# esw0116/DynaVSR

Hardware: AMD Instinct MI355X
Metric: inner-loop frames/sec/GPU (EDVR-M x4, 5x3x180x320): forward leg = BASELINE.json configs[1]; the inner MAML step and the per-frame pipeline are `inner_step` / `per_frame_pipeline` (higher is better)
Workload: dtype f32; 1 GPU; EDVR-M x4 forward (PCD deformable alignment + TSA fusion + reconstruction), clips of 1x5x3x180x320 -> 3x720x1280 (BASELINE.json configs[1]); one step = 2 clip(s) per GPU, one per HIP stream (adapt.super_resolve_video); clips_in_flight_per_gpu=2

## Files before the change

### dynavsr_amd/_lib.py

```python
import ctypes
import os
from ctypes import POINTER, Structure, c_char_p, c_float, c_int, c_longlong, c_size_t, c_void_p

import torch

_runtime = {"configured": False, "hw_queues": None, "effective": None}


def configure_runtime(hw_queues=6):
    if not _runtime["configured"]:
        user = os.environ.get("GPU_MAX_HW_QUEUES")
        late = torch.cuda.is_initialized()
        if user is None and not late:
            os.environ["GPU_MAX_HW_QUEUES"] = str(int(hw_queues))
        _runtime.update(configured=True, hw_queues=os.environ.get("GPU_MAX_HW_QUEUES"),
                        effective=(user is not None) or not late)
    return {"hw_queues": _runtime["hw_queues"], "effective": _runtime["effective"]}


def runtime_report(device=None):
    r = configure_runtime()
    overlaps = None
    if torch.cuda.is_available():
        with torch.cuda.device(device if device is not None else torch.cuda.current_device()):
# ... 126 lines not shown
        "dvsr_avgpool2_backward": (I, [P, P, LL, I, I, I, P]),
        "dvsr_resize_bilinear_ac_forward": (I, [P, P, LL, I, I, I, I, F, LL, P]),
        "dvsr_resize_bilinear_ac_backward": (I, [P, P, LL, I, I, I, I, F, LL, P]),
        "dvsr_upsample_bicubic_ac_forward": (I, [P, P, LL, I, I, I, P]),
        "dvsr_upsample_bicubic_ac_backward": (I, [P, P, LL, I, I, I, P]),
        "dvsr_channel_affine": (I, [P, P, P, P, I, I, LL, LL, LL, I, P]),
        "dvsr_batchnorm_workspace_bytes": (c_size_t, [I]),
        "dvsr_batchnorm_forward": (I, [P] * 8 + [I, I, LL, I, F, F, I, P, c_size_t, P]),
        "dvsr_batchnorm_backward": (I, [P] * 9 + [I, I, LL, I, I, P, c_size_t, P]),
        "dvsr_temporal_gather3_forward": (I, [P, P, I, I, I, LL, I, P]),
        "dvsr_temporal_gather3_backward": (I, [P, P, I, I, I, LL, I, P]),
        "dvsr_dynamic_filter_forward": (I, [P, P, P, P, I, I, I, I, I, P]),
        "dvsr_dynamic_filter_backward": (I, [P, P, P, P, P, P, I, I, I, I, I, P]),
        "dvsr_conv3x3_small_cout": (I, [P, P, P, P, P, I, I, I, I, I, I, P]),
        "dvsr_conv1x1_dual": (I, [P, P, P, P, P, P, P, I, I, I, I, I, P]),
        "dvsr_patch_gather_forward": (I, [P, P, POINTER(c_int), POINTER(c_int), I, I, I, I, I, I, P]),
        "dvsr_patch_gather_backward": (I, [P, P, POINTER(c_int), POINTER(c_int), I, I, I, I, I, I, P]),
        "dvsr_l1_tail_forward": (I, [P, P, P, F, P, LL, P, c_size_t, P]),
        "dvsr_l1_tail_backward": (I, [P, P, P, F, P, LL, P]),
        "dvsr_charbonnier_backward": (I, [P, P, P, P, LL, F, P]),
        "dvsr_charbonnier_forward_grouped": (I, [P, P, P, LL, I, F, P, c_size_t, P]),
        "dvsr_charbonnier_backward_grouped": (I, [P, P, P, P, LL, I, F, P]),
        "dvsr_l1_tail_forward_grouped": (I, [P, P, P, F, P, LL, I, P, c_size_t, P]),
        "dvsr_l1_tail_backward_grouped": (I, [P, P, P, F, P, LL, I, P]),
        "dvsr_edvr_op_info": (I, [P, I, c_char_p, I, c_char_p, I, POINTER(ctypes.c_double),
                                  POINTER(ctypes.c_double)]),
        "dvsr_edvr_forward_timed": (I, [P, POINTER(c_void_p), P, P, P, c_size_t, P, POINTER(c_float)]),
        "dvsr_debug_mfma_peak": (LL, [P, I, I, I, I, P]),
        "dvsr_debug_mfma_shadow": (I, [P, P, I, I, I, I, I, P]),
        "dvsr_edvr_tensor_info": (I, [P, c_char_p, POINTER(LL), POINTER(LL)]),
        "dvsr_edvr_plan_work": (I, [P, POINTER(ctypes.c_double * 9)]),
        "dvsr_edvr_plan_work_nograd": (I, [P, POINTER(ctypes.c_double * 9)]),
        "dvsr_edvr_op_launch_count": (I, [P, I, I]),
        "dvsr_side_stream_overlaps": (I, [P]),
        "dvsr_edvr_op_output": (I, [P, I, I, POINTER(c_int), POINTER(LL), POINTER(LL)]),
        "dvsr_estimator_plan_work": (I, [P, POINTER(ctypes.c_double * 9)]),
        "dvsr_edvr_stream_create": (I, [POINTER(EdvrConfig), I, I, I, POINTER(c_void_p)]),
        "dvsr_edvr_stream_destroy": (None, [P]),
        "dvsr_edvr_stream_num_params": (I, [P]),
        "dvsr_edvr_stream_num_launches": (I, [P, I]),
        "dvsr_edvr_stream_cache_bytes": (c_size_t, [P]),
        "dvsr_edvr_stream_workspace_bytes": (c_size_t, [P]),
        "dvsr_edvr_stream_extract": (I, [P, POINTER(c_void_p), P, I, P, c_size_t, P, c_size_t, I, P]),
        "dvsr_edvr_stream_fuse": (I, [P, POINTER(c_void_p), POINTER(c_int), P, c_size_t, P, P, c_size_t, I, P]),
        "dvsr_frame_ingest": (I, [P, POINTER(FrameDesc), P, I, I, I, P]),
        "dvsr_frame_emit": (I, [P, I, I, P, POINTER(FrameDesc), F, F, P]),
        "dvsr_edvr_stream_extract_frame": (I, [P, POINTER(c_void_p), P, POINTER(FrameDesc), I, I, P, c_size_t, P, c_size_t, I,
                                               P]),
# ... 54 lines not shown
```

### dynavsr_amd/csrc/engine.hip

```cpp
#include <algorithm>
#include <cstdlib>
#include <string>
#include <vector>

#include "common.h"
#include "kernels.h"
#include "small_grid.h"

namespace dvsr {

enum { SP_ARENA = 0, SP_INPUT = 1, SP_OUTPUT = 2, SP_NONE = 3 };
struct T {
  int space = SP_NONE;
  size_t off = 0, numel = 0;
  bool valid() const { return space != SP_NONE; }
};

enum OpType { OP_CONV, OP_DCN, OP_UP, OP_POOL, OP_GATE, OP_BLEND, OP_ADD, OP_PAD, OP_MEANSUB, OP_ADDMEAN };

struct Op {
  OpType type;
  const char* name = "";
  T x0, x1, res, y, y2;
  int pw = -1, pb = -1;
// ... 13 lines not shown
  float mul = 1.f;
  size_t planes = 0;
  int gB = 0, gN = 0, gC = 0;
  size_t gHW = 0;
  struct PackSlot { ConvGeo geo = {8, 8, 2}; size_t off = 0, floats = 0; };
  PackSlot dgrad[2], dcn_pack;
  enum LaunchRole { WHOLE, MAIN_PART, REF_PART };
  struct Launch { PackSlot pack; int c_off = 0, c = 0; LaunchRole role = WHOLE; };
  struct LaunchList {
    int n = 0; Launch l[2];
    const Launch* begin() const { return l; }
    const Launch* end() const { return l + n; }
    const Launch& primary() const { return l[n - 1]; }
  } launches[2];
  struct T pre;
};
enum FwdMode { FWD_GRAD = 0, FWD_NOGRAD = 1 };

enum { R_ACT = 0, R_GRAD = 1, R_X = 2, R_GX = 3, R_GOUT = 4, R_TMP = 5, R_NONE = 6 };
struct Ref {
  int space = R_NONE;
  size_t off = 0;
};
enum BType { B_MEMSET, B_COPYADD, B_ACT, B_WGRAD, B_DGRAD, B_REDUCE, B_DCN, B_UP, B_POOL, B_GATE, B_BLEND,
             B_PADFOLD, B_ADDMEAN, B_WUNMAP };
struct BOp {
  BType type;
  int fwd = -1;
  Ref a, b, c, d, e, f;
  size_t n = 0;
// ... 110 lines not shown
    if (g5.kernel == ConvKernel::WINO_F4) nograd.l[0] = whole(g5);
  }
  const Op::LaunchList pair = plan_hoist(o, p, fwd_ok, nograd.l[0]);
  if (pair.n) {
    o.pre = arena_alloc(p, "", (size_t)(N / o.x1_bdiv) * Cout * Ho * Wo);
    nograd = pair;
  }
  for (int which = 0; which < 2; ++which) {
    const int ci = which ? c1 : c0;
    if (!ci) continue;
    Op::PackSlot& dg = o.dgrad[which];
    dg.geo = as_bf(conv2_choose(ks, 1, N, o.H, o.W, ci, Cout, (!o.ps && o.stride == 1) ? ks_ok : ALLOW_NONE), o.H, o.W, ci, true);
    dg.floats = conv2_pack_floats(ks, ci, Cout, dg.geo);
    dg.off = p.dpack_floats;
    p.dpack_floats += dg.floats * p.wsets;
  }
}

struct Builder {
  dvsr_edvr_plan& p;
  int pcur = 0;
  explicit Builder(dvsr_edvr_plan& plan) : p(plan) {}

  T alloc(const char* name, size_t numel) { return arena_alloc(p, name, numel); }
  static T view(const T& base, size_t off, size_t numel) {
    T t = base;
    t.off += off;
    t.numel = numel;
    return t;
  }
// ... 147 lines not shown
  T emb = b.conv("tsa_emb", tA1, aligned, C, none, 0, BN, H, W, C, 3, 1, NO);
  T cor = b.alloc("tsa_cor", (size_t)BN * HW);
  T gated = b.alloc("tsa_gated", (size_t)BN * C * HW);
  {
    Op o; o.type = OP_GATE; o.name = "tsa_gate"; o.x0 = emb; o.x1 = emb_ref; o.res = aligned;
    o.y = cor; o.y2 = gated; o.gB = B; o.gN = Nf; o.gC = C; o.gHW = HW;
    p.ops.push_back(o);
  }
  T fea = b.conv("tsa_fea", ffu, gated, Nf * C, none, 0, B, H, W, C, 1, 1, L);
  T att = b.conv("tsa_att1", s1, gated, Nf * C, none, 0, B, H, W, C, 1, 1, L);
  {
    static const bool dual_on = [] { const char* v = getenv("DVSR_TSA_DUAL"); return !(v && v[0] == '0'); }();
    const int ia = (int)p.ops.size() - 2, ib = ia + 1;
    if (dual_on && C == 64 && !p.cfg.bf16_mfma) { p.ops[ia].dual = ib; p.ops[ib].fused_into = ia; }
  }
  T pmx, pav;
  b.pool("tsa_pool1", att, (size_t)B * C, H, W, pmx, pav);
  att = b.conv("tsa_att2", s2, pmx, C, pav, C, B, H2, W2, C, 1, 1, L);
  T attL = b.conv("tsa_attL1", sL1, att, C, none, 0, B, H2, W2, C, 1, 1, L);
  T qmx, qav;
  b.pool("tsa_pool2", attL, (size_t)B * C, H2, W2, qmx, qav);
  attL = b.conv("tsa_attL2", sL2, qmx, C, qav, C, B, H4, W4, C, 3, 1, L);
  attL = b.conv("tsa_attL3", sL3, attL, C, none, 0, B, H4, W4, C, 3, 1, L);
  T attLu = b.up("tsa_attL_up", attL, (size_t)B * C, H4, W4, 2, 1.f);
  T a3 = b.conv("tsa_att3", s3, att, C, none, 0, B, H2, W2, C, 3, 1, L);
  T att3 = b.alloc("tsa_att3_sum", (size_t)B * C * HW2);
  {
    Op o; o.type = OP_ADD; o.name = "tsa_att3_add"; o.x0 = a3; o.x1 = attLu; o.y = att3;
    p.ops.push_back(o);
  }
  T a4 = b.conv("tsa_att4", s4, att3, C, none, 0, B, H2, W2, C, 1, 1, L);
  T a4u = b.up("tsa_att4_up", a4, (size_t)B * C, H2, W2, 2, 1.f);
  T a5 = b.conv("tsa_att", s5, a4u, C, none, 0, B, H, W, C, 3, 1, NO);
  T ad = b.conv("tsa_add1", sa1, a5, C, none, 0, B, H, W, C, 1, 1, L);
  ad = b.conv("tsa_add2", sa2, ad, C, none, 0, B, H, W, C, 1, 1, NO);
  T out = b.alloc("tsa_out", (size_t)B * C * HW);
  {
    Op o; o.type = OP_BLEND; o.name = "tsa_blend"; o.x0 = fea; o.x1 = a5; o.res = ad; o.y = out;
    p.ops.push_back(o);
  }

  for (int i = 0; i < c.back_RBs; ++i) {
    auto p1 = b.take(); auto p2 = b.take();
    T t = b.conv("rc_rb_a", p1, out, C, none, 0, B, H, W, C, 3, 1, R);
    out = b.conv("rc_rb_b", p2, t, C, none, 0, B, H, W, C, 3, 1, NO, out);
  }
  p.named.emplace_back("recon", out);
  int h = H, w = W;
  if (c.scale == 4) {
    out = b.conv("upconv1", b.take(), out, C, none, 0, B, h, w, C * 4, 3, 1, L, none, 2);
    h *= 2; w *= 2;
    out = b.conv("upconv2", b.take(), out, C, none, 0, B, h, w, 256, 3, 1, L, none, 2);
  } else {
    out = b.conv("upconv2", b.take(), out, C, none, 0, B, h, w, 256, 3, 1, L, none, 2);
  }
// ... 431 lines not shown
        }
      }
    }
  }
  return flush();
}

static dvsr_conv2d_desc launch_desc(dvsr_conv2d_desc d, const Op& o, Op::LaunchRole role, float* pre) {
  if (role == Op::WHOLE) return d;
  if (role == Op::REF_PART) { d.x0 = d.x1; d.c0 = o.c1; d.x0_bstride = o.x1_bs; d.N = o.N / o.x1_bdiv; d.act = ACT_NONE; d.y = pre; }
  else { d.bias = nullptr; d.pre = pre; d.pre_bdiv = o.x1_bdiv; }
  d.x1 = nullptr; d.c1 = 0; d.x1_bdiv = 1; d.x1_bstride = 0;
  return d;
}

static int run_forward_op(const dvsr_edvr_plan& p, const Op& o, const float* const* P, const Bases& bs, hipStream_t st) {
  switch (o.type) {
    case OP_CONV: {
      dvsr_conv2d_desc d = {};
      d.x0 = bs.at(o.x0); d.x1 = bs.at(o.x1); d.w = P[o.pw]; d.bias = P[o.pb]; d.res = bs.at(o.res);
      d.y = bs.at(o.y);
      d.N = o.N; d.c0 = o.c0; d.c1 = o.c1; d.H = o.H; d.W = o.W; d.Cout = o.Cout; d.ks = o.ks;
      d.stride = o.stride; d.pad = conv_pad(o); d.act = o.act; d.pixel_shuffle = o.ps;
      if (o.pad_out) { d.y = bs.at(o.ypad); d.pixel_shuffle = o.pad_out; }
      if (!p.use_v1 && (o.dual >= 0 || o.fused_into >= 0)) {
        const Op& oa = o.dual >= 0 ? o : p.ops[o.fused_into];
        const Op& ob = p.ops[oa.dual];
        const long long HW = (long long)oa.H * oa.W;
        auto plain1x1 = [](const Op& q) {
          return q.type == OP_CONV && q.ks == 1 && q.stride == 1 && q.c1 == 0 && q.Cout == 64 && !q.res.valid() && !q.ps && !q.wmap && !q.pad_out;
        };
// ... 310 lines not shown
  {
    const ConvGeo& g = p->ops[index].launches[FWD_NOGRAD].primary().pack.geo;
    snprintf(name, name_cap, "%s[%d/%d/%d%s]", p->ops[index].name, g.cc, g.th, g.mt, kernel_tag(g.kernel));
  }
  else
    snprintf(name, name_cap, "%s", p->ops[index].name);
  return DVSR_OK;
}

extern "C" int dvsr_edvr_op_launch_count(const dvsr_edvr_plan* p, int index, int nograd) {
  if (!p || index < 0 || index >= (int)p->ops.size()) return -1;
  const Op& o = p->ops[index];
  return o.type == OP_CONV ? o.launches[nograd ? FWD_NOGRAD : FWD_GRAD].n : 1;
}

static int plan_work(const dvsr_edvr_plan* p, double* out9, FwdMode mode) {
  DVSR_REQUIRE(p && out9, DVSR_ERR_INVALID, "edvr_plan_work: null argument");
  double fa = 0, fe = 0, ba = 0, be = 0, fby = 0, f32p[2] = {0, 0}, bfp[2] = {0, 0};
  auto conv_part = [](const Op& o, int ci) {
    return 2.0 * (double)o.N * conv_out(o, o.H) * conv_out(o, o.W) * o.Cout * ci * o.ks * o.ks;
  };
  auto issue = [&](const ConvGeo& g, double f, double* ex, int pass) {
    const double shaped = f * multiplies_per_output_ratio(g.kernel);
    *ex += shaped;
    if (on_bf16_split(g.kernel) || g.bf == 2) bfp[pass] += 6.0 * shaped;
    else if (g.bf == 1) bfp[pass] += shaped;
    else f32p[pass] += shaped;
  };
  for (const Op& o : p->ops) {
    {
      const char* k; double fl, by;
      op_work(o, &k, &fl, &by);
      fby += by;
    }
    if (o.type == OP_CONV) {
      const double f = conv_part(o, o.c0 + o.c1);
      fa += f;
      for (const Op::Launch& l : o.launches[mode])
        issue(l.pack.geo, conv_part(o, l.c) / (l.role == Op::REF_PART ? o.x1_bdiv : 1), &fe, 0);
    } else if (o.type == OP_DCN) {
      const double f = 2.0 * (double)o.N * o.H * o.W * o.Cout * o.c0 * 9;
      fa += f; fe += f; f32p[0] += f;
    }
  }
  for (const BOp& b : p->bops) {
    if (b.fwd < 0) continue;
    const Op& o = p->ops[b.fwd];
// ... 407 lines not shown
```

### dynavsr_amd/csrc/kernels.h

```cpp
#pragma once
#include "../../include/dynavsr_hip.h"
#include "common.h"

namespace dvsr {

struct ConvExtra {
  int wt = 0;
  int w_ctot = 0, w_coff = 0;
  int in_ps = 0;
  int in_dil = 0, Hs = 0, Ws = 0;
  int accum = 0;
  const float* gmask = nullptr;
  int gmask_act = 0;
  int wdiv = 1; long long w_gs = 0; int b_gs = 0;
};
int conv2d_run(const dvsr_conv2d_desc& d, const ConvExtra& ex, hipStream_t st);

int mdcn_forward_run(const float* x, const float* off, long long off_bs, const float* msk,
                     long long msk_bs, int mask_logit, const float* w, const float* b, float* out,
                     int N, int C, int H, int W, int Cout, int kh, int kw, int stride, int pad,
                     int dil, int groups, int dg, int act, hipStream_t st);

enum class ConvKernel : int {
  REG = 0,
// ... 57 lines not shown
  return conv2_pack_entry(w, P, ks, Cout, Ctot, g.cc, g.bf, pack_layout(g.kernel), wt, w_ctot, w_coff);
}
double conv2_f4_occupied_cycles(int N, int Ho, int Wo, int Cout, int Ctot, int th);
int pack_weights_wino_run(const PackTable& t, hipStream_t st);
int pack_weights_wino3_run(const PackTable& t, hipStream_t st);
int pack_weights_wino5_run(const PackTable& t, hipStream_t st);
int conv2d_packed_run(const dvsr_conv2d_desc& d, const float* wp, const ConvExtra& ex, const ConvGeo& geo,
                      hipStream_t st);

bool conv1x1_dual_ok(const float* x, const float* w0, const float* w1, const float* y0, const float* y1, int Cin, long long HW);
int conv1x1_dual_run(const float* x, const float* w0, const float* b0, const float* w1, const float* b1, float* y0, float* y1,
                     int N, int Cin, int HW, int act, hipStream_t st, int wdiv = 1, long long w_gs = 0, int b_gs = 0);
int conv3x3_small_cout_run(const float* x, const float* w, const float* bias, const float* res, float* y, int N,
                           int C, int H, int W, int Cout, int act, hipStream_t st, int wdiv = 1, long long w_gs = 0,
                           int b_gs = 0);

struct WgradReduceEntry {
  float* partial; float* dbp; float* dW; float* db;
  int nslot, KK, OP, CP, Cout, Cin, Ctot, c_off;
  int ngroups = 1;
  long long dW_gs = 0, db_gs = 0;
};
constexpr int WGRAD_REDUCE_BATCH = 44;
struct WgradReduceTable {
  int n;
  WgradReduceEntry e[WGRAD_REDUCE_BATCH];
};
int wgrad_reduce_batch(const WgradReduceEntry* entries, int n, hipStream_t st, int blocks = 96);
struct WgradDesc {
  const float* x = nullptr; long long x_bs = 0; int x_bdiv = 1;
// ... 143 lines not shown
```

### dynavsr_amd/engine.py

```python
import ctypes
import threading

import torch

from . import _lib as L

_plans = {}
_GEOMETRY_ENV = ("DVSR_CONV_WINO", "DVSR_CONV_WINO3", "DVSR_CONV_WINO5", "DVSR_CONV_V1", "DVSR_EST_SPLIT", "DVSR_EST_SPLIT2", "DVSR_FUSE_ACT_BWD",
                 "DVSR_BWD_STREAMS", "DVSR_PCD_HOIST")
_PROCESS_ENV = ("DVSR_CONV_LDS", "DVSR_CONV_LAST_MFMA", "DVSR_SPLIT_TH8_FROM", "DVSR_WGRAD_SPLIT3",
                "DVSR_WGRAD_WIDE", "DVSR_WGRAD_S3V", "DVSR_WGRAD_S3_KYS_BELOW", "DVSR_WGRAD_S3_WGS", "DVSR_WGRAD_S3W", "DVSR_DCN_FWD", "DVSR_DCN_BWD",
                "DVSR_EST_FUSE_PAD", "DVSR_FUSE_RES_BWD", "DVSR_BWD_FORK_EVERY", "DVSR_BWD_PROBE", "DVSR_TSA_DUAL", "DVSR_TSA_V",
                "DVSR_DEGRADE_GENERIC", "DVSR_UP2")
_process_env_seen = None


def _check_process_env():
    import os
    import warnings
    global _process_env_seen
    now = tuple(os.environ.get(k) for k in _PROCESS_ENV)
    if _process_env_seen is None:
        _process_env_seen = now
        return
# ... 63 lines not shown
        L.check(L.lib().dvsr_edvr_op_output(self._h, index, which, ctypes.byref(ia), ctypes.byref(off), ctypes.byref(n)),
                "dvsr_edvr_op_output")
        if not ia.value:
            return None
        return ws.view(torch.float32)[off.value:off.value + n.value]

    def op_info(self):
        out = []
        kind, name = ctypes.create_string_buffer(32), ctypes.create_string_buffer(64)
        fl, by = ctypes.c_double(), ctypes.c_double()
        for i in range(self.n_launches):
            L.check(L.lib().dvsr_edvr_op_info(self._h, i, kind, 32, name, 64, ctypes.byref(fl),
                                              ctypes.byref(by)), "dvsr_edvr_op_info")
            out.append((kind.value.decode(), name.value.decode(), fl.value, by.value))
        return out

    def tensor(self, ws, name, shape=None):
        off, n = ctypes.c_longlong(), ctypes.c_longlong()
        L.check(L.lib().dvsr_edvr_tensor_info(self._h, name.encode(), ctypes.byref(off),
                                              ctypes.byref(n)), "dvsr_edvr_tensor_info")
        t = ws.view(torch.float32)[off.value:off.value + n.value]
        return t.view(shape) if shape is not None else t

    def __del__(self):
        try:
            if self._h:
                L.lib().dvsr_edvr_plan_destroy(self._h)
        except Exception:
            pass

# ... 415 lines not shown
```

### include/dynavsr_hip.h

```cpp
#ifndef DYNAVSR_HIP_H_
#define DYNAVSR_HIP_H_

#include <stddef.h>

#ifdef __cplusplus
extern "C" {
#endif

#define DVSR_OK 0
#define DVSR_ERR_INVALID (-1)
#define DVSR_ERR_UNSUPPORTED (-2)
#define DVSR_ERR_WORKSPACE (-3)
#define DVSR_ERR_HIP (-4)

#define DVSR_ACT_NONE 0
#define DVSR_ACT_LRELU 1
#define DVSR_ACT_RELU 2

typedef void* dvsr_stream_t;

const char* dvsr_last_error(void);
int dvsr_version(void);

int dvsr_mdcn_forward(const float* x, const float* offset, const float* mask, const float* w,
// ... 78 lines not shown
int dvsr_edvr_num_launches(const dvsr_edvr_plan* plan);
size_t dvsr_edvr_workspace_bytes(const dvsr_edvr_plan* plan, int need_grad);
int dvsr_edvr_forward(const dvsr_edvr_plan* plan, const float* const* params, const float* x,
                      float* out, void* workspace, size_t workspace_bytes, dvsr_stream_t stream);
int dvsr_edvr_forward_packed(const dvsr_edvr_plan* plan, const float* const* params, const float* x,
                             float* out, void* workspace, size_t workspace_bytes, dvsr_stream_t stream);
int dvsr_edvr_backward(const dvsr_edvr_plan* plan, const float* const* params, const float* x,
                       const float* grad_out, float* const* grad_params, float* grad_x, void* workspace,
                       size_t workspace_bytes, dvsr_stream_t stream);
int dvsr_edvr_num_backward_launches(const dvsr_edvr_plan* plan);
int dvsr_edvr_op_info(const dvsr_edvr_plan* plan, int index, char* kind, int kind_cap, char* name,
                      int name_cap, double* flops, double* bytes);
int dvsr_edvr_plan_work(const dvsr_edvr_plan* plan, double* out9);
int dvsr_edvr_plan_work_nograd(const dvsr_edvr_plan* plan, double* out9);
int dvsr_edvr_op_launch_count(const dvsr_edvr_plan* plan, int index, int nograd);
int dvsr_side_stream_overlaps(dvsr_stream_t stream);
int dvsr_edvr_op_output(const dvsr_edvr_plan* plan, int index, int which, int* in_arena, long long* offset_floats,
                        long long* numel);
int dvsr_edvr_forward_timed(const dvsr_edvr_plan* plan, const float* const* params, const float* x,
                            float* out, void* workspace, size_t workspace_bytes,
                            dvsr_stream_t stream, float* op_ms);
long long dvsr_debug_mfma_peak(float* out, int blocks, int iters, int nacc, int lds_bytes, dvsr_stream_t stream);
int dvsr_debug_mfma_shadow(long long* cycles, float* out, int blocks, int iters, int nv, int kind, int acc,
                           dvsr_stream_t stream);
int dvsr_edvr_tensor_info(const dvsr_edvr_plan* plan, const char* name, long long* offset_floats,
                          long long* numel);

#define DVSR_STREAM_MAX_FRAMES 16
typedef struct dvsr_edvr_stream dvsr_edvr_stream;
int dvsr_edvr_stream_create(const dvsr_edvr_config* cfg, int H, int W, int slots, dvsr_edvr_stream** out);
// ... 175 lines not shown
                                  dvsr_stream_t stream);
int dvsr_temporal_gather3_backward(const float* grad_y, float* grad_x, int B, int T, int C, long long HW, int pad_t,
                                   dvsr_stream_t stream);
int dvsr_dynamic_filter_forward(const float* x_center, const float* filter_logits, const float* residual, float* out,
                                int B, int H, int W, int scale, int adapt_official, dvsr_stream_t stream);
int dvsr_dynamic_filter_backward(const float* x_center, const float* filter_logits, const float* grad_out,
                                 float* grad_logits, float* grad_residual, float* grad_x_center, int B, int H, int W,
                                 int scale, int adapt_official, dvsr_stream_t stream);

int dvsr_conv3x3_small_cout(const float* x, const float* w, const float* bias, const float* res, float* y, int N, int C, int H,
                            int W, int Cout, int act, dvsr_stream_t stream);

int dvsr_conv1x1_dual(const float* x, const float* w0, const float* b0, const float* w1, const float* b1, float* y0, float* y1,
                      int N, int Cin, int H, int W, int act, dvsr_stream_t stream);

int dvsr_patch_gather_forward(const float* src, float* dst, const int* py, const int* px, int P, int planes, int H, int W,
                              int edge, int scale, dvsr_stream_t stream);
int dvsr_patch_gather_backward(const float* grad_dst, float* grad_src, const int* py, const int* px, int P, int planes,
                               int H, int W, int edge, int scale, dvsr_stream_t stream);

int dvsr_adam_step(float* const* params, const float* const* grads, float* const* exp_avg,
                   float* const* exp_avg_sq, const long long* numel, int n_tensors, float lr, float beta1,
                   float beta2, float eps, float weight_decay, int step, dvsr_stream_t stream);
int dvsr_sgd_step(float* const* params, const float* const* grads, const long long* numel, int n_tensors,
                  float lr, float weight_decay, dvsr_stream_t stream);
int dvsr_replicate_tensors(const float* const* src, float* const* dst, const long long* numel, int n_tensors, int copies,
                           dvsr_stream_t stream);

size_t dvsr_frame_metrics_workspace_bytes(int C, int H, int W);
int dvsr_frame_metrics(const float* sr, const float* gt, int C, int H, int W, float lo, float hi,
// ... 11 lines not shown
```

Before: 266.0 frames/s.

## Fuse TSA pool/attention, upsample-add/attention and tail convs into MFMA kernels

Adds three fused HIP kernels for the TSA fusion module. The first does pool plus two 1x1 convs, the second does bilinear upsample-add plus a 1x1 conv, and the third does the add1/add2 1x1 convs plus the sigmoid blend. The planner marks the absorbed ops and, in no-grad forward mode, launches one fused kernel per chain instead of several separate ones. The aim is to cut launches and the round trips of intermediate activations through global memory. It only applies for nf=64, fp32 and aligned shapes, can be turned off with DVSR_TSA_FUSE=0, and leaves the grad forward path unchanged.

```diff
diff --git a/dynavsr_amd/_lib.py b/dynavsr_amd/_lib.py
--- a/dynavsr_amd/_lib.py
+++ b/dynavsr_amd/_lib.py
@@ -164,6 +164,9 @@
         "dvsr_dynamic_filter_backward": (I, [P, P, P, P, P, P, I, I, I, I, I, P]),
         "dvsr_conv3x3_small_cout": (I, [P, P, P, P, P, I, I, I, I, I, I, P]),
         "dvsr_conv1x1_dual": (I, [P, P, P, P, P, P, P, I, I, I, I, I, P]),
+        "dvsr_tsa_pool_att": (I, [P, P, P, P, P, P, P, I, I, I, P]),
+        "dvsr_tsa_up_add_att": (I, [P, P, P, P, P, I, I, I, P]),
+        "dvsr_tsa_tail": (I, [P, P, P, P, P, P, P, I, I, I, P]),
         "dvsr_patch_gather_forward": (I, [P, P, POINTER(c_int), POINTER(c_int), I, I, I, I, I, I, P]),
         "dvsr_patch_gather_backward": (I, [P, P, POINTER(c_int), POINTER(c_int), I, I, I, I, I, I, P]),
         "dvsr_l1_tail_forward": (I, [P, P, P, F, P, LL, P, c_size_t, P]),
@@ -182,6 +185,7 @@
         "dvsr_edvr_plan_work": (I, [P, POINTER(ctypes.c_double * 9)]),
         "dvsr_edvr_plan_work_nograd": (I, [P, POINTER(ctypes.c_double * 9)]),
         "dvsr_edvr_op_launch_count": (I, [P, I, I]),
+        "dvsr_edvr_op_absorbed_by": (I, [P, I]),
         "dvsr_side_stream_overlaps": (I, [P]),
         "dvsr_edvr_op_output": (I, [P, I, I, POINTER(c_int), POINTER(LL), POINTER(LL)]),
         "dvsr_estimator_plan_work": (I, [P, POINTER(ctypes.c_double * 9)]),
diff --git a/dynavsr_amd/csrc/engine.hip b/dynavsr_amd/csrc/engine.hip
--- a/dynavsr_amd/csrc/engine.hip
+++ b/dynavsr_amd/csrc/engine.hip
@@ -51,6 +51,8 @@
     const Launch& primary() const { return l[n - 1]; }
   } launches[2];
   struct T pre;
+  enum TsaChain { CHAIN_NONE = 0, CHAIN_POOL_ATT, CHAIN_UP_ADD_ATT, CHAIN_TAIL };
+  int tsa_chain = CHAIN_NONE, absorbed_by = -1, chain_ops[2] = {-1, -1};
 };
 enum FwdMode { FWD_GRAD = 0, FWD_NOGRAD = 1 };
 
@@ -191,6 +193,29 @@
     dg.floats = conv2_pack_floats(ks, ci, Cout, dg.geo);
     dg.off = p.dpack_floats;
     p.dpack_floats += dg.floats * p.wsets;
+  }
+}
+
+static bool tsa_chain_applies(const dvsr_edvr_plan& p, Op::TsaChain which) {
+  const char* v = getenv("DVSR_TSA_FUSE");
+  if ((v && v[0] == '0') || p.use_v1 || p.wsets != 1 || p.cfg.nf != 64 || p.cfg.bf16_mfma || p.H % 4 != 0 || p.W % 4 != 0) return false;
+  return which != Op::CHAIN_UP_ADD_ATT || (p.W / 4) % 4 == 0;
+}
+static void plan_tsa_chain(dvsr_edvr_plan& p, Op::TsaChain which, int a, int b, int last) {
+  if (!tsa_chain_applies(p, which)) return;
+  p.ops[last].tsa_chain = which;
+  p.ops[last].chain_ops[0] = a; p.ops[last].chain_ops[1] = b;
+  p.ops[a].absorbed_by = p.ops[b].absorbed_by = p.ops[last].absorbed_by = last;
+}
+static double tsa_chain_bytes(const dvsr_edvr_plan& p, const Op& last) {
+  const Op& a = p.ops[last.chain_ops[0]];
+  const Op& b = p.ops[last.chain_ops[1]];
+  auto wts = [](const Op& c) { return (double)c.Cout * (c.c0 + c.c1); };
+  switch (last.tsa_chain) {
+    case Op::CHAIN_POOL_ATT: return 4.0 * ((double)a.planes * a.H * a.W + (double)b.y.numel + (double)last.y.numel + wts(b) + wts(last));
+    case Op::CHAIN_UP_ADD_ATT: return 4.0 * ((double)a.planes * a.H * a.W + (double)b.x0.numel + (double)last.y.numel + wts(last));
+    case Op::CHAIN_TAIL: return 4.0 * (3.0 * last.y.numel + wts(a) + wts(b));
+    default: return 0.0;
   }
 }
 
@@ -368,15 +393,19 @@
     const int ia = (int)p.ops.size() - 2, ib = ia + 1;
     if (dual_on && C == 64 && !p.cfg.bf16_mfma) { p.ops[ia].dual = ib; p.ops[ib].fused_into = ia; }
   }
+  auto last_op = [&]() { return (int)p.ops.size() - 1; };
   T pmx, pav;
   b.pool("tsa_pool1", att, (size_t)B * C, H, W, pmx, pav);
+  const int i_pool1 = last_op();
   att = b.conv("tsa_att2", s2, pmx, C, pav, C, B, H2, W2, C, 1, 1, L);
   T attL = b.conv("tsa_attL1", sL1, att, C, none, 0, B, H2, W2, C, 1, 1, L);
+  plan_tsa_chain(p, Op::CHAIN_POOL_ATT, i_pool1, last_op() - 1, last_op());
   T qmx, qav;
   b.pool("tsa_pool2", attL, (size_t)B * C, H2, W2, qmx, qav);
   attL = b.conv("tsa_attL2", sL2, qmx, C, qav, C, B, H4, W4, C, 3, 1, L);
   attL = b.conv("tsa_attL3", sL3, attL, C, none, 0, B, H4, W4, C, 3, 1, L);
   T attLu = b.up("tsa_attL_up", attL, (size_t)B * C, H4, W4, 2, 1.f);
+  const int i_attL_up = last_op();
   T a3 = b.conv("tsa_att3", s3, att, C, none, 0, B, H2, W2, C, 3, 1, L);
   T att3 = b.alloc("tsa_att3_sum", (size_t)B * C * HW2);
   {
@@ -384,6 +413,7 @@
     p.ops.push_back(o);
   }
   T a4 = b.conv("tsa_att4", s4, att3, C, none, 0, B, H2, W2, C, 1, 1, L);
+  plan_tsa_chain(p, Op::CHAIN_UP_ADD_ATT, i_attL_up, last_op() - 1, last_op());
   T a4u = b.up("tsa_att4_up", a4, (size_t)B * C, H2, W2, 2, 1.f);
   T a5 = b.conv("tsa_att", s5, a4u, C, none, 0, B, H, W, C, 3, 1, NO);
   T ad = b.conv("tsa_add1", sa1, a5, C, none, 0, B, H, W, C, 1, 1, L);
@@ -393,6 +423,7 @@
     Op o; o.type = OP_BLEND; o.name = "tsa_blend"; o.x0 = fea; o.x1 = a5; o.res = ad; o.y = out;
     p.ops.push_back(o);
   }
+  plan_tsa_chain(p, Op::CHAIN_TAIL, last_op() - 2, last_op() - 1, last_op());
 
   for (int i = 0; i < c.back_RBs; ++i) {
     auto p1 = b.take(); auto p2 = b.take();
@@ -854,7 +885,36 @@
   return d;
 }
 
+static int tsa_chain_launch(const dvsr_edvr_plan& p, const Op& last, const float* const* P, const Bases& bs, hipStream_t st, bool run,
+                            bool* ok) {
+  const Op& a = p.ops[last.chain_ops[0]];
+  const Op& b = p.ops[last.chain_ops[1]];
+  switch (last.tsa_chain) {
+    case Op::CHAIN_POOL_ATT:
+      *ok = tsa_pool_att_ok(P[b.pw], P[last.pw], b.Cout, a.H, a.W);
+      return run ? tsa_pool_att_run(bs.at(a.x0), P[b.pw], P[b.pb], P[last.pw], P[last.pb], bs.at(b.y), bs.at(last.y), b.N, a.H, a.W, st)
+                 : DVSR_OK;
+    case Op::CHAIN_UP_ADD_ATT:
+      *ok = tsa_up_add_att_ok(bs.at(a.x0), P[last.pw], last.Cout, last.H, last.W);
+      return run ? tsa_up_add_att_run(bs.at(b.x0), bs.at(a.x0), P[last.pw], P[last.pb], bs.at(last.y), last.N, last.H, last.W, st)
+                 : DVSR_OK;
+    case Op::CHAIN_TAIL:
+      *ok = tsa_tail_ok(bs.at(a.x0), bs.at(last.x0), P[a.pw], P[b.pw], bs.at(last.y), a.Cout, (long long)a.H * a.W);
+      return run ? tsa_tail_run(bs.at(a.x0), bs.at(last.x0), P[a.pw], P[a.pb], P[b.pw], P[b.pb], bs.at(last.y), a.N, a.H * a.W, st)
+                 : DVSR_OK;
+    default:
+      *ok = false;
+      return DVSR_OK;
+  }
+}
+
 static int run_forward_op(const dvsr_edvr_plan& p, const Op& o, const float* const* P, const Bases& bs, hipStream_t st) {
+  if (bs.mode == FWD_NOGRAD && o.absorbed_by >= 0) {
+    const Op& last = p.ops[o.absorbed_by];
+    bool ok = false;
+    (void)tsa_chain_launch(p, last, P, bs, st, false, &ok);
+    if (ok) return &o == &last ? tsa_chain_launch(p, last, P, bs, st, true, &ok) : DVSR_OK;
+  }
   switch (o.type) {
     case OP_CONV: {
       dvsr_conv2d_desc d = {};
@@ -1195,6 +1255,11 @@
   return o.type == OP_CONV ? o.launches[nograd ? FWD_NOGRAD : FWD_GRAD].n : 1;
 }
 
+extern "C" int dvsr_edvr_op_absorbed_by(const dvsr_edvr_plan* p, int index) {
+  if (!p || index < 0 || index >= (int)p->ops.size()) return -2;
+  return p->ops[index].absorbed_by;
+}
+
 static int plan_work(const dvsr_edvr_plan* p, double* out9, FwdMode mode) {
   DVSR_REQUIRE(p && out9, DVSR_ERR_INVALID, "edvr_plan_work: null argument");
   double fa = 0, fe = 0, ba = 0, be = 0, fby = 0, f32p[2] = {0, 0}, bfp[2] = {0, 0};
@@ -1212,6 +1277,7 @@
     {
       const char* k; double fl, by;
       op_work(o, &k, &fl, &by);
+      if (mode == FWD_NOGRAD && o.absorbed_by >= 0) by = &o == &p->ops[o.absorbed_by] ? tsa_chain_bytes(*p, o) : 0.0;
       fby += by;
     }
     if (o.type == OP_CONV) {
diff --git a/dynavsr_amd/csrc/kernels.h b/dynavsr_amd/csrc/kernels.h
--- a/dynavsr_amd/csrc/kernels.h
+++ b/dynavsr_amd/csrc/kernels.h
@@ -95,6 +95,16 @@
 int conv3x3_small_cout_run(const float* x, const float* w, const float* bias, const float* res, float* y, int N,
                            int C, int H, int W, int Cout, int act, hipStream_t st, int wdiv = 1, long long w_gs = 0,
                            int b_gs = 0);
+
+bool tsa_pool_att_ok(const float* w2, const float* wl, int C, int H, int W);
+int tsa_pool_att_run(const float* x, const float* w2, const float* b2, const float* wl, const float* bl, float* att, float* attl,
+                     int N, int H, int W, hipStream_t st);
+bool tsa_up_add_att_ok(const float* al, const float* w, int C, int H, int W);
+int tsa_up_add_att_run(const float* a3, const float* al, const float* w, const float* b, float* y, int N, int H, int W,
+                       hipStream_t st);
+bool tsa_tail_ok(const float* a5, const float* fea, const float* w1, const float* w2, const float* out, int C, long long HW);
+int tsa_tail_run(const float* a5, const float* fea, const float* w1, const float* b1, const float* w2, const float* b2,
+                 float* out, int N, int HW, hipStream_t st);
 
 struct WgradReduceEntry {
   float* partial; float* dbp; float* dW; float* db;
diff --git a/dynavsr_amd/csrc/tsa_fused.hip b/dynavsr_amd/csrc/tsa_fused.hip
--- /dev/null
+++ b/dynavsr_amd/csrc/tsa_fused.hip
@@ -0,0 +1,306 @@
+#include "common.h"
+#include "kernels.h"
+
+namespace dvsr {
+namespace {
+
+constexpr int TF_C = 64;
+
+template <int K>
+__device__ __forceinline__ void load_w_row(const float* __restrict__ w, int co, int hi, float (&a)[K / 2]) {
+#pragma unroll
+  for (int m = 0; m < K / 4; ++m) {
+    const f32x4 v = *reinterpret_cast<const f32x4*>(w + (size_t)co * K + 4 * m);
+    a[2 * m] = hi ? v[1] : v[0];
+    a[2 * m + 1] = hi ? v[3] : v[2];
+  }
+}
+
+__device__ __forceinline__ int acc_row(int r, int hi) { return (r & 3) + 8 * (r >> 2) + 4 * hi; }
+
+__device__ __forceinline__ void load_bias(const float* __restrict__ b, int cw, int hi, float (&bv)[16]) {
+#pragma unroll
+  for (int r = 0; r < 16; ++r) bv[r] = b ? b[cw + acc_row(r, hi)] : 0.f;
+}
+
+template <int K, int NJ, int PITCH>
+__device__ __forceinline__ void contract(const float* s, const float (&a)[K / 2], f32x16 (&acc)[NJ]) {
+#pragma unroll
+  for (int j = 0; j < NJ; ++j)
+#pragma unroll
+    for (int r = 0; r < 16; ++r) acc[j][r] = 0.f;
+#pragma unroll
+  for (int i = 0; i < K / 2; ++i) {
+    if constexpr (NJ == 2) {
+      const f32x2 b = *reinterpret_cast<const f32x2*>(s + 2 * i * PITCH);
+      acc[0] = __builtin_amdgcn_mfma_f32_32x32x2f32(a[i], b[0], acc[0], 0, 0, 0);
+      acc[1] = __builtin_amdgcn_mfma_f32_32x32x2f32(a[i], b[1], acc[1], 0, 0, 0);
+    } else {
+      acc[0] = __builtin_amdgcn_mfma_f32_32x32x2f32(a[i], s[2 * i * PITCH], acc[0], 0, 0, 0);
+    }
+  }
+}
+
+__device__ __forceinline__ float lrelu(float v) { return fmaxf(v, 0.1f * v); }
+
+constexpr int TP_PX = 64;
+
+struct TsaPoolAttK {
+  const float* x; const float* w2; const float* b2; const float* wl; const float* bl; float* att; float* attl;
+  int H, W, Ho, Wo, tiles_per_img;
+};
+
+__global__ __launch_bounds__(256) void tsa_pool_att_kernel(TsaPoolAttK a) {
+  __shared__ __attribute__((aligned(16))) float s_x[2 * TF_C * TP_PX];
+  __shared__ __attribute__((aligned(16))) float s_t[TF_C * TP_PX];
+  const int tile = blockIdx.x;
+  const int n = tile / a.tiles_per_img, p0 = (tile - n * a.tiles_per_img) * TP_PX;
+  const int tid = threadIdx.x, lane = tid & 63;
+  const int wave = __builtin_amdgcn_readfirstlane(tid >> 6);
+  const int nn = lane & 31, hi = lane >> 5, cw = (wave & 1) * 32, ph = wave >> 1;
+  const int HWo = a.Ho * a.Wo;
+
+  float a2[TF_C], al[TF_C / 2], bv2[16], bvl[16];
+  load_w_row<2 * TF_C>(a.w2, cw + nn, hi, a2);
+  load_w_row<TF_C>(a.wl, cw + nn, hi, al);
+  load_bias(a.b2, cw, hi, bv2);
+  load_bias(a.bl, cw, hi, bvl);
+
+  {
+    const int pl = tid & 63;
+    const int p = min(p0 + pl, HWo - 1);
+    const int oy = p / a.Wo, ox = p - oy * a.Wo;
+    int toff[9];
+    bool tin[9];
+#pragma unroll
+    for (int t = 0; t < 9; ++t) {
+      const int yy = 2 * oy + t / 3 - 1, xx = 2 * ox + t % 3 - 1;
+      tin[t] = (unsigned)yy < (unsigned)a.H && (unsigned)xx < (unsigned)a.W;
+      toff[t] = min(max(yy, 0), a.H - 1) * a.W + min(max(xx, 0), a.W - 1);
+    }
+    const float* xn = a.x + (size_t)n * TF_C * a.H * a.W;
+#pragma unroll 4
+    for (int k = 0; k < TF_C / 4; ++k) {
+      const int c = (tid >> 6) + 4 * k;
+      const float* pln = xn + (size_t)c * a.H * a.W;
+      float v[9];
+#pragma unroll
+      for (int t = 0; t < 9; ++t) v[t] = pln[toff[t]];
+      float mx = -INFINITY, sum = 0.f;
+#pragma unroll
+      for (int t = 0; t < 9; ++t) {
+        mx = fmaxf(mx, tin[t] ? v[t] : -INFINITY);
+        sum += tin[t] ? v[t] : 0.f;
+      }
+      s_x[c * TP_PX + pl] = mx;
+      s_x[(TF_C + c) * TP_PX + pl] = sum * (1.f / 9.f);
+    }
+  }
+  __syncthreads();
+
+  const int col = ph * 32 + nn, px = p0 + col;
+  const bool live = px < HWo;
+  f32x16 acc[1];
+  contract<2 * TF_C, 1, TP_PX>(s_x + hi * TP_PX + col, a2, acc);
+  float* yb = a.att + (size_t)n * TF_C * HWo + px;
+#pragma unroll
+  for (int r = 0; r < 16; ++r) {
+    const int co = cw + acc_row(r, hi);
+    const float v = lrelu(acc[0][r] + bv2[r]);
+    s_t[co * TP_PX + col] = v;
+    if (live) yb[(size_t)co * HWo] = v;
+  }
+  __syncthreads();
+  contract<TF_C, 1, TP_PX>(s_t + hi * TP_PX + col, al, acc);
+  yb = a.attl + (size_t)n * TF_C * HWo + px;
+  if (live) {
+#pragma unroll
+    for (int r = 0; r < 16; ++r) yb[(size_t)(cw + acc_row(r, hi)) * HWo] = lrelu(acc[0][r] + bvl[r]);
+  }
+}
+
+struct TsaUpAddAttK {
+  const float* a3; const float* al; const float* w; const float* b; float* y;
+  int H, W, tiles_per_img;
+};
+
+__global__ __launch_bounds__(256) void tsa_up_add_att_kernel(TsaUpAddAttK a) {
+  __shared__ __attribute__((aligned(16))) float s_x[TF_C * TP_PX];
+  const int tile = blockIdx.x;
+  const int n = tile / a.tiles_per_img, p0 = (tile - n * a.tiles_per_img) * TP_PX;
+  const int tid = threadIdx.x, lane = tid & 63;
+  const int wave = __builtin_amdgcn_readfirstlane(tid >> 6);
+  const int nn = lane & 31, hi = lane >> 5, cw = (wave & 1) * 32, ph = wave >> 1;
+  const int HW = a.H * a.W, Hs = a.H >> 1, Ws = a.W >> 1;
+
+  float aw[TF_C / 2], bv[16];
+  load_w_row<TF_C>(a.w, cw + nn, hi, aw);
+  load_bias(a.b, cw, hi, bv);
+
+  {
+    const int pl = tid & 63;
+    const int p = min(p0 + pl, HW - 1);
+    const int oy = p / a.W, ox = p - oy * a.W;
+    const int iy = oy >> 1, ix = ox >> 1;
+    const int yu = iy > 0 ? iy - 1 : 0, yd = iy < Hs - 1 ? iy + 1 : Hs - 1;
+    const int xl = ix > 0 ? ix - 1 : 0, xr = ix < Ws - 1 ? ix + 1 : Ws - 1;
+    const bool oddx = ox & 1, oddy = oy & 1;
+    auto blend = [](float near, float far) { return __fmaf_rn(0.25f, far, __fmul_rn(0.75f, near)); };
+    const int xf = oddx ? xr : xl, yf = oddy ? yd : yu;
+    const bool copyx = !oddx && ix == 0, copyy = !oddy && iy == 0;
+    const int o_nn = iy * Ws + ix, o_nf = iy * Ws + xf, o_fn = yf * Ws + ix, o_ff = yf * Ws + xf;
+    const float* a3n = a.a3 + (size_t)n * TF_C * HW + p;
+    const float* aln = a.al + (size_t)n * TF_C * Hs * Ws;
+#pragma unroll 8
+    for (int k = 0; k < TF_C / 4; ++k) {
+      const int c = (tid >> 6) + 4 * k;
+      const float* pln = aln + (size_t)c * Hs * Ws;
+      const float v_nn = pln[o_nn], v_nf = pln[o_nf], v_fn = pln[o_fn], v_ff = pln[o_ff], base = a3n[(size_t)c * HW];
+      const float hn = copyx ? v_nn : blend(v_nn, v_nf), hf = copyx ? v_fn : blend(v_fn, v_ff);
+      const float up = copyy ? hn : blend(hn, hf);
+      s_x[c * TP_PX + pl] = base + up;
+    }
+  }
+  __syncthreads();
+
+  const int col = ph * 32 + nn, px = p0 + col;
+  f32x16 acc[1];
+  contract<TF_C, 1, TP_PX>(s_x + hi * TP_PX + col, aw, acc);
+  if (px < HW) {
+    float* yb = a.y + (size_t)n * TF_C * HW + px;
+#pragma unroll
+    for (int r = 0; r < 16; ++r) yb[(size_t)(cw + acc_row(r, hi)) * HW] = lrelu(acc[0][r] + bv[r]);
+  }
+}
+
+constexpr int TT_PX = 128;
+
+struct TsaTailK {
+  const float* a5; const float* fea; const float* w1; const float* b1; const float* w2; const float* b2; float* out;
+  int HW, tiles_per_img;
+};
+
+__global__ __launch_bounds__(256, 2) void tsa_tail_kernel(TsaTailK a) {
+  __shared__ __attribute__((aligned(16))) float s_x[TF_C * TT_PX];
+  __shared__ __attribute__((aligned(16))) float s_t[TF_C * TT_PX];
+  const int tile = blockIdx.x;
+  const int n = tile / a.tiles_per_img, p0 = (tile - n * a.tiles_per_img) * TT_PX;
+  const int tid = threadIdx.x, lane = tid & 63;
+  const int wave = __builtin_amdgcn_readfirstlane(tid >> 6);
+  const int nn = lane & 31, hi = lane >> 5, cw = (wave & 1) * 32, ph = wave >> 1;
+  const size_t img = (size_t)n * TF_C * a.HW;
+
+  {
+    const float* xn = a.a5 + img;
+    f32x4 v[8];
+#pragma unroll
+    for (int e = 0; e < 8; ++e) {
+      const int idx = tid + 256 * e, c = idx >> 5, px = min(p0 + 4 * (idx & 31), a.HW - 4);
+      v[e] = *reinterpret_cast<const f32x4*>(xn + (size_t)c * a.HW + px);
+    }
+#pragma unroll
+    for (int e = 0; e < 8; ++e) *reinterpret_cast<f32x4*>(&s_x[4 * (tid + 256 * e)]) = v[e];
+  }
+  float a1[TF_C / 2], a2[TF_C / 2], bv1[16], bv2[16];
+  load_w_row<TF_C>(a.w1, cw + nn, hi, a1);
+  load_w_row<TF_C>(a.w2, cw + nn, hi, a2);
+  load_bias(a.b1, cw, hi, bv1);
+  load_bias(a.b2, cw, hi, bv2);
+  __syncthreads();
+
+  const int col = ph * 64 + 2 * nn, px = p0 + col;
+  const bool live = px < a.HW;
+  f32x16 acc[2];
+  contract<TF_C, 2, TT_PX>(s_x + hi * TT_PX + col, a1, acc);
+#pragma unroll
+  for (int r = 0; r < 16; ++r)
+    *reinterpret_cast<f32x2*>(&s_t[(cw + acc_row(r, hi)) * TT_PX + col]) = f32x2{lrelu(acc[0][r] + bv1[r]), lrelu(acc[1][r] + bv1[r])};
+  __syncthreads();
+
+  f32x2 fv[16];
+  const float* fb = a.fea + img + (live ? px : 0);
+#pragma unroll
+  for (int r = 0; r < 16; ++r) fv[r] = *reinterpret_cast<const f32x2*>(fb + (size_t)(cw + acc_row(r, hi)) * a.HW);
+  contract<TF_C, 2, TT_PX>(s_t + hi * TT_PX + col, a2, acc);
+  if (!live) return;
+  float* ob = a.out + img + px;
+#pragma unroll
+  for (int r = 0; r < 16; ++r) {
+    const int co = cw + acc_row(r, hi);
+    const f32x2 att = *reinterpret_cast<const f32x2*>(&s_x[co * TT_PX + col]);
+    f32x2 o;
+#pragma unroll
+    for (int j = 0; j < 2; ++j) {
+      const float add = acc[j][r] + bv2[r];
+      o[j] = fv[r][j] * sigmoidf_(att[j]) * 2.f + add;
+    }
+    *reinterpret_cast<f32x2*>(ob + (size_t)co * a.HW) = o;
+  }
+}
+
+bool aligned16(std::initializer_list<const void*> ps) {
+  uintptr_t m = 0;
+  for (const void* p : ps) m |= (uintptr_t)p;
+  return (m & 15) == 0;
+}
+
+}
+
+bool tsa_pool_att_ok(const float* w2, const float* wl, int C, int H, int W) {
+  return C == TF_C && H >= 2 && W >= 2 && H % 2 == 0 && W % 2 == 0 && (long long)H * W < (1ll << 28) && aligned16({w2, wl});
+}
+int tsa_pool_att_run(const float* x, const float* w2, const float* b2, const float* wl, const float* bl, float* att, float* attl,
+                     int N, int H, int W, hipStream_t st) {
+  DVSR_REQUIRE(x && w2 && wl && att && attl && N > 0, DVSR_ERR_INVALID, "tsa_pool_att: bad argument");
+  DVSR_REQUIRE(tsa_pool_att_ok(w2, wl, TF_C, H, W), DVSR_ERR_UNSUPPORTED, "tsa_pool_att: H=%d W=%d / alignment", H, W);
+  TsaPoolAttK k;
+  k.x = x; k.w2 = w2; k.b2 = b2; k.wl = wl; k.bl = bl; k.att = att; k.attl = attl;
+  k.H = H; k.W = W; k.Ho = H / 2; k.Wo = W / 2; k.tiles_per_img = ceil_div(k.Ho * k.Wo, TP_PX);
+  hipLaunchKernelGGL(tsa_pool_att_kernel, dim3(N * k.tiles_per_img), dim3(256), 0, st, k);
+  return check_launch("tsa_pool_att_kernel");
+}
+
+bool tsa_up_add_att_ok(const float* al, const float* w, int C, int H, int W) {
+  return C == TF_C && H >= 2 && W >= 2 && H % 2 == 0 && W % 2 == 0 && (long long)H * W < (1ll << 28) && aligned16({al, w});
+}
+int tsa_up_add_att_run(const float* a3, const float* al, const float* w, const float* b, float* y, int N, int H, int W,
+                       hipStream_t st) {
+  DVSR_REQUIRE(a3 && al && w && y && N > 0, DVSR_ERR_INVALID, "tsa_up_add_att: bad argument");
+  DVSR_REQUIRE(tsa_up_add_att_ok(al, w, TF_C, H, W), DVSR_ERR_UNSUPPORTED, "tsa_up_add_att: H=%d W=%d / alignment", H, W);
+  TsaUpAddAttK k;
+  k.a3 = a3; k.al = al; k.w = w; k.b = b; k.y = y; k.H = H; k.W = W; k.tiles_per_img = ceil_div(H * W, TP_PX);
+  hipLaunchKernelGGL(tsa_up_add_att_kernel, dim3(N * k.tiles_per_img), dim3(256), 0, st, k);
+  return check_launch("tsa_up_add_att_kernel");
+}
+
+bool tsa_tail_ok(const float* a5, const float* fea, const float* w1, const float* w2, const float* out, int C, long long HW) {
+  return C == TF_C && HW % 4 == 0 && HW >= 4 && HW < (1ll << 28) && aligned16({a5, fea, w1, w2, out});
+}
+int tsa_tail_run(const float* a5, const float* fea, const float* w1, const float* b1, const float* w2, const float* b2,
+                 float* out, int N, int HW, hipStream_t st) {
+  DVSR_REQUIRE(a5 && fea && w1 && w2 && out && N > 0, DVSR_ERR_INVALID, "tsa_tail: bad argument");
+  DVSR_REQUIRE(tsa_tail_ok(a5, fea, w1, w2, out, TF_C, HW), DVSR_ERR_UNSUPPORTED, "tsa_tail: HW=%d / alignment", HW);
+  TsaTailK k;
+  k.a5 = a5; k.fea = fea; k.w1 = w1; k.b1 = b1; k.w2 = w2; k.b2 = b2; k.out = out; k.HW = HW;
+  k.tiles_per_img = ceil_div(HW, TT_PX);
+  hipLaunchKernelGGL(tsa_tail_kernel, dim3(N * k.tiles_per_img), dim3(256), 0, st, k);
+  return check_launch("tsa_tail_kernel");
+}
+
+}
+
+extern "C" int dvsr_tsa_pool_att(const float* x, const float* w2, const float* b2, const float* wl, const float* bl, float* att,
+                                 float* attl, int N, int H, int W, dvsr_stream_t stream) {
+  return dvsr::tsa_pool_att_run(x, w2, b2, wl, bl, att, attl, N, H, W, (hipStream_t)stream);
+}
+
+extern "C" int dvsr_tsa_up_add_att(const float* a3, const float* al, const float* w, const float* b, float* y, int N, int H,
+                                   int W, dvsr_stream_t stream) {
+  return dvsr::tsa_up_add_att_run(a3, al, w, b, y, N, H, W, (hipStream_t)stream);
+}
+
+extern "C" int dvsr_tsa_tail(const float* a5, const float* fea, const float* w1, const float* b1, const float* w2,
+                             const float* b2, float* out, int N, int H, int W, dvsr_stream_t stream) {
+  DVSR_REQUIRE(N > 0 && H > 0 && W > 0, DVSR_ERR_INVALID, "tsa_tail: empty tensor");
+  return dvsr::tsa_tail_run(a5, fea, w1, b1, w2, b2, out, N, H * W, (hipStream_t)stream);
+}
diff --git a/dynavsr_amd/engine.py b/dynavsr_amd/engine.py
--- a/dynavsr_amd/engine.py
+++ b/dynavsr_amd/engine.py
@@ -7,7 +7,7 @@
 
 _plans = {}
 _GEOMETRY_ENV = ("DVSR_CONV_WINO", "DVSR_CONV_WINO3", "DVSR_CONV_WINO5", "DVSR_CONV_V1", "DVSR_EST_SPLIT", "DVSR_EST_SPLIT2", "DVSR_FUSE_ACT_BWD",
-                 "DVSR_BWD_STREAMS", "DVSR_PCD_HOIST")
+                 "DVSR_BWD_STREAMS", "DVSR_PCD_HOIST", "DVSR_TSA_FUSE")
 _PROCESS_ENV = ("DVSR_CONV_LDS", "DVSR_CONV_LAST_MFMA", "DVSR_SPLIT_TH8_FROM", "DVSR_WGRAD_SPLIT3",
                 "DVSR_WGRAD_WIDE", "DVSR_WGRAD_S3V", "DVSR_WGRAD_S3_KYS_BELOW", "DVSR_WGRAD_S3_WGS", "DVSR_WGRAD_S3W", "DVSR_DCN_FWD", "DVSR_DCN_BWD",
                 "DVSR_EST_FUSE_PAD", "DVSR_FUSE_RES_BWD", "DVSR_BWD_FORK_EVERY", "DVSR_BWD_PROBE", "DVSR_TSA_DUAL", "DVSR_TSA_V",
@@ -101,6 +101,9 @@
                                               ctypes.byref(by)), "dvsr_edvr_op_info")
             out.append((kind.value.decode(), name.value.decode(), fl.value, by.value))
         return out
+
+    def absorbed_by(self):
+        return [int(L.lib().dvsr_edvr_op_absorbed_by(self._h, i)) for i in range(self.n_launches)]
 
     def tensor(self, ws, name, shape=None):
         off, n = ctypes.c_longlong(), ctypes.c_longlong()
diff --git a/include/dynavsr_hip.h b/include/dynavsr_hip.h
--- a/include/dynavsr_hip.h
+++ b/include/dynavsr_hip.h
@@ -116,6 +116,7 @@
 int dvsr_edvr_plan_work(const dvsr_edvr_plan* plan, double* out9);
 int dvsr_edvr_plan_work_nograd(const dvsr_edvr_plan* plan, double* out9);
 int dvsr_edvr_op_launch_count(const dvsr_edvr_plan* plan, int index, int nograd);
+int dvsr_edvr_op_absorbed_by(const dvsr_edvr_plan* plan, int index);
 int dvsr_side_stream_overlaps(dvsr_stream_t stream);
 int dvsr_edvr_op_output(const dvsr_edvr_plan* plan, int index, int which, int* in_arena, long long* offset_floats,
                         long long* numel);
@@ -321,6 +322,13 @@
 int dvsr_conv1x1_dual(const float* x, const float* w0, const float* b0, const float* w1, const float* b1, float* y0, float* y1,
                       int N, int Cin, int H, int W, int act, dvsr_stream_t stream);
 
+int dvsr_tsa_pool_att(const float* x, const float* w2, const float* b2, const float* wl, const float* bl, float* att,
+                      float* attl, int N, int H, int W, dvsr_stream_t stream);
+int dvsr_tsa_up_add_att(const float* a3, const float* al, const float* w, const float* b, float* y, int N, int H, int W,
+                        dvsr_stream_t stream);
+int dvsr_tsa_tail(const float* a5, const float* fea, const float* w1, const float* b1, const float* w2, const float* b2,
+                  float* out, int N, int H, int W, dvsr_stream_t stream);
+
 int dvsr_patch_gather_forward(const float* src, float* dst, const int* py, const int* px, int P, int planes, int H, int W,
                               int edge, int scale, dvsr_stream_t stream);
 int dvsr_patch_gather_backward(const float* grad_dst, float* grad_src, const int* py, const int* px, int P, int planes,
```

Result: no change. 267.4 frames/s, median of 6 (+0.5%).
